# google/kubeflow

Measured on AMD Instinct MI355X. Metric: pytorchjob_train_tokens_per_s, higher is better.
Workload: dtype bf16; 1 GPU; model=llama3-8b, global_batch=7, seq_len=4096, parallelism=dp1

## Files before the change

### kubeflow_amd/ops/_backend.py

```python
from __future__ import annotations

import ctypes
import os
from pathlib import Path

_LIB_PATH = Path(__file__).resolve().parent / "libkfops.so"
_lib = None
_load_error: str | None = None


def native_enabled() -> bool:
    return os.environ.get("KF_NATIVE_KERNELS", "1") != "0"


def try_load():
    global _lib, _load_error
    if _lib is not None:
        return _lib
    if not native_enabled():
        _load_error = "disabled via KF_NATIVE_KERNELS=0"
        return None
    from . import build_ext
    if build_ext.needs_build():
        try:
# ... 27 lines not shown
_FP = ctypes.POINTER(ctypes.c_float)
_PI64 = ctypes.POINTER(ctypes.c_int64)
_PI32 = ctypes.POINTER(ctypes.c_int32)

_DQ8 = [_P] * 5 + [_FP, _FP] + [_I64] * 7 + [_F, _I32]
_DKV8 = [_P] + _DQ8
_ROPE_TAIL = [_FP, _FP, _I64]
_BWD_HEAD = [_P] * 8 + [_FP, _FP] + [_I64] * 4
_ATTN_BWD = _BWD_HEAD + [_I64] * 5 + [_F, _I32]
_ATTN_FWD = [_P, _FP, _P, _P, _P] + [_I64] * 7 + [_F, _I32, _P]

SIGNATURES: dict[str, list] = {
    "kf_rmsnorm_fwd": [_P, _FP, _P, _P, _I64, _I64, _F, _P],
    "kf_rmsnorm_bwd_nparts": [_I64],
    "kf_rmsnorm_bwd": [_P, _P, _FP, _P, _P, _P, _FP, _I64, _I64, _P],
    "kf_rmsnorm_bwd_res": [_P, _P, _FP, _P, _P, _P, _FP, _P, _I64, _I64, _P],
    "kf_layernorm_fwd": [_P, _FP, _FP, _P, _P, _P, _I64, _I64, _F, _P],
    "kf_layernorm_bwd_nparts": [_I64],
    "kf_layernorm_bwd": [_P, _P, _P, _FP, _P, _P, _P, _FP, _FP, _I64, _I64,
                         _P],
    "kf_rope": [_P, _P, _FP, _FP, _PI64] + [_I64] * 8 + [_I32, _P],
    "kf_swiglu_fwd": [_P, _P, _I64, _I64, _P],
    "kf_swiglu_bwd": [_P, _P, _P, _I64, _I64, _P],
    "kf_adamw": [_P, _FP, _P, _FP, _FP, _FP, _I64, _F, _F, _F, _F, _F, _I64,
                 _P],
    "kf_adamw_clip": [_P, _FP, _P, _FP, _FP, _FP, _P, _FP, _I64, _F, _F, _F,
                      _F, _F, _I64, _P],
    "kf_grad_sumsq_nparts": [_I64],
    "kf_grad_sumsq": [_FP, _FP, _P, _I64, _P],
    "kf_ce_fwd": [_FP, _FP, _P, _PI64, _I64, _I64, _I64, _P],
    "kf_ce_bwd": [_P, _P, _FP, _PI64, _FP, _I64, _I64, _I64, _P],
    "kf_skinny_gemm": [_P, _P, _P, _P] + [_I64] * 6 + [_P],
    "kf_skinny_gemm_q8": [_P, _P, _P, _FP, _P] + [_I64] * 6 + [_P],
    "kf_skinny_gemm_grouped": [_P, _P, _P, _PI32, _PI32] + [_I64] * 6 + [_P],
    "kf_skinny_gemm_grouped_q8": [_P, _P, _P, _FP, _PI32, _PI32] +
                                 [_I64] * 6 + [_P],
    "kf_kv_store": [_P] * 6 + [_I64, _I64, _I64, _P],
    "kf_decode_rope_store": [_P, _P, _P, _P, _FP, _FP, _PI32, _P] +
                            [_I64] * 5 + [_P],
    "kf_attn_fwd": _ATTN_FWD,
    "kf_attn_fwd4": _ATTN_FWD,
    "kf_attn_fwd4_rect": [_P, _FP, _P, _P, _P] + [_I64] * 8 + [_F, _I64, _P],
    "kf_attn_fwd4_abl": [_I32] + _ATTN_FWD,
    "kf_tr16_probe": [_P, _P, _I32, _P],
    "kf_attn_bwd": _ATTN_BWD + [_P],
    "kf_attn_bwd_rope": _ATTN_BWD + _ROPE_TAIL + [_P],
    "kf_attn_bwd8_dq": _DQ8 + [_P],
    "kf_attn_bwd8_dq_rope": _DQ8 + _ROPE_TAIL + [_P],
    "kf_attn_bwd8_dkv": _DKV8 + [_P],
    "kf_attn_bwd8_dkv_rope": _DKV8 + _ROPE_TAIL + [_P],
    "kf_attn_bwd8_dkv_fused": _DKV8 + [_P],
    "kf_attn_bwd8_dkv_fused_rope": _DKV8 + _ROPE_TAIL + [_P],
    "kf_attn64_fwd": [_P, _FP, _P, _P, _P] + [_I64] * 6 + [_F, _I32, _I64,
                                                           _P],
    "kf_attn64_bwd": _BWD_HEAD + [_I64, _I64, _F, _I32, _I64, _P],
    "kf_attn64_fwd_varlen": [_P, _FP, _P, _P, _P, _PI32] + [_I64] * 6 +
                            [_F, _P],
    "kf_attn64_bwd_varlen": _BWD_HEAD[:10] + [_PI32] + [_I64] * 6 + [_F, _P],
    "kf_attn_decode": [_P] * 6 + [_PI32, _PI32] + [_I64] * 6 + [_F, _P],
    "kf_moe_route": [_P, _FP, _P, _P, _I64, _I64, _I64, _P],
    "kf_moe_route_bwd": [_P, _P, _FP, _P, _I64, _I64, _I64, _P],
    "kf_moe_sort_nwork": [_I64, _I64, _I64],
    "kf_moe_sort": [_P] * 5 + [_I64] * 4 + [_P],
    "kf_moe_gather": [_P, _P, _P, _I64, _I64, _I64, _P],
    "kf_moe_gather_bwd": [_P, _P, _P] + [_I64] * 4 + [_P],
    "kf_moe_combine": [_P] * 4 + [_I64] * 4 + [_P],
    "kf_moe_combine_bwd": [_P] * 6 + [_I64] * 4 + [_P],
}
_RETURNS_INT64 = ("kf_rmsnorm_bwd_nparts", "kf_layernorm_bwd_nparts",
# ... 19 lines not shown
```

### kubeflow_amd/ops/csrc/attention_bwd.hip

```cpp

#include "kf_attn_common.h"

#define AB_D 128

__global__ __launch_bounds__(256) void kf_attn_delta2_kernel(
    float* __restrict__ delta, const unsigned short* __restrict__ dout,
    const unsigned short* __restrict__ o, int64_t B, int S, int Hq) {
  const int64_t nrows = B * (int64_t)S * Hq;
  const int wid = threadIdx.x / KF_WAVE;
  const int lane = threadIdx.x & (KF_WAVE - 1);
  for (int64_t row = blockIdx.x * 4 + wid; row < nrows; row += gridDim.x * 4) {
    const unsigned short* dor = dout + row * AB_D;
    const unsigned short* orow = o + row * AB_D;
    kf_short4 a = *reinterpret_cast<const kf_short4*>(dor + lane * 2);
    kf_short4 bv = *reinterpret_cast<const kf_short4*>(orow + lane * 2);
    float s = kf_bf16_to_f32((unsigned short)a[0]) *
                  kf_bf16_to_f32((unsigned short)bv[0]) +
              kf_bf16_to_f32((unsigned short)a[1]) *
                  kf_bf16_to_f32((unsigned short)bv[1]);
    s = kf_wave_sum(s);
    if (lane == 0) {
      const int h = (int)(row % Hq);
      const int64_t bs = row / Hq;
      const int64_t b = bs / S;
      const int st = (int)(bs % S);
      delta[(b * Hq + h) * (int64_t)S + st] = s;
    }
  }
}

#define DQ_KT 64

__global__ __launch_bounds__(256) void kf_attn_dq_kernel(
    unsigned short* __restrict__ dq, const unsigned short* __restrict__ q,
    const unsigned short* __restrict__ k, const unsigned short* __restrict__ v,
    const unsigned short* __restrict__ dout, const float* __restrict__ lse,
    const float* __restrict__ delta, int64_t B, int S, int Hq, int Hkv,
    int64_t qts, int64_t kts, int64_t dqts, float scale, int causal) {
  __shared__ unsigned char k_lds[DQ_KT * AB_D * 2];
  __shared__ unsigned char v_lds[DQ_KT * AB_D * 2];
  __shared__ unsigned char kt_lds[AB_D * DQ_KT * 2];
  __shared__ unsigned char ds_lds[4][16 * DQ_KT * 2];
// ... 243 lines not shown
      for (int nt = 0; nt < 8; ++nt) {
        kf_bf16x8 dob = *reinterpret_cast<const kf_bf16x8*>(
            dot_lds + kf_swz(nt * 16 + l16, lg * 16, 64));
        dvacc[nt] =
            __builtin_amdgcn_mfma_f32_16x16x32_bf16(ptf, dob, dvacc[nt], 0, 0, 0);
        kf_bf16x8 qb = *reinterpret_cast<const kf_bf16x8*>(
            qt_lds + kf_swz(nt * 16 + l16, lg * 16, 64));
        dkacc[nt] =
            __builtin_amdgcn_mfma_f32_16x16x32_bf16(dstf, qb, dkacc[nt], 0, 0, 0);
      }
    }
  }

  const int krow0 = kt * 64 + w * 16 + lg * 4;
#pragma unroll
  for (int r = 0; r < 4; ++r) {
    const int64_t base = (b * S + krow0 + r) * dkts + (int64_t)hkv * AB_D;
#pragma unroll
    for (int nt = 0; nt < 8; ++nt) {
      dk[base + nt * 16 + l16] = kf_f32_to_bf16(dkacc[nt][r]);
      dv[base + nt * 16 + l16] = kf_f32_to_bf16(dvacc[nt][r]);
    }
  }
}

KF_EXPORT int kf_attn_bwd(void* dq, void* dk, void* dv, const void* dout,
                          const void* q, const void* k, const void* v,
                          const void* o, const float* lse, float* delta,
                          int64_t B, int64_t S, int64_t Hq, int64_t Hkv,
                          int64_t D, int64_t qts, int64_t kts, int64_t dqts,
                          int64_t dkts, float scale, int causal,
                          void* stream) {
  return kf_attn_bwd_rope(dq, dk, dv, dout, q, k, v, o, lse, delta, B, S, Hq,
                          Hkv, D, qts, kts, dqts, dkts, scale, causal,
                          nullptr, nullptr, 0, stream);
}

KF_EXPORT int kf_attn_bwd_rope(void* dq, void* dk, void* dv, const void* dout,
                               const void* q, const void* k, const void* v,
                               const void* o, const float* lse, float* delta,
                               int64_t B, int64_t S, int64_t Hq, int64_t Hkv,
                               int64_t D, int64_t qts, int64_t kts,
                               int64_t dqts, int64_t dkts, float scale,
                               int causal, const float* cost,
                               const float* sint, int64_t pos_offset,
                               void* stream) {
  if (D != AB_D || S % 64 || Hq % Hkv) return (int)hipErrorInvalidValue;
  if ((cost == nullptr) != (sint == nullptr)) return (int)hipErrorInvalidValue;
  if (qts == 0) qts = Hq * AB_D;
  if (kts == 0) kts = Hkv * AB_D;
  if (dqts == 0) dqts = Hq * AB_D;
  if (dkts == 0) dkts = Hkv * AB_D;
  hipLaunchKernelGGL(kf_attn_delta2_kernel,
                     dim3(kf_grid_for(B * S * Hq, 4)), dim3(256), 0,
                     (hipStream_t)stream, delta, (const unsigned short*)dout,
                     (const unsigned short*)o, B, (int)S, (int)Hq);
  int err = (int)hipGetLastError();
  if (err) return err;
  if (S % 256 == 0) {
    err = kf_attn_bwd8_dq_rope(dq, q, k, v, dout, lse, delta, B, S, Hq, Hkv,
                               qts, kts, dqts, scale, causal, cost, sint,
                               pos_offset, stream);
    if (err) return err;
    return kf_attn_bwd8_dkv_fused_rope(dk, dv, q, k, v, dout, lse, delta, B,
                                       S, Hq, Hkv, qts, kts, dkts, scale,
                                       causal, cost, sint, pos_offset,
                                       stream);
  }
  dim3 gq((unsigned)(S / 64), (unsigned)Hq, (unsigned)B);
  hipLaunchKernelGGL(kf_attn_dq_kernel, gq, dim3(256), 0, (hipStream_t)stream,
                     (unsigned short*)dq, (const unsigned short*)q,
                     (const unsigned short*)k, (const unsigned short*)v,
                     (const unsigned short*)dout, lse, delta, B, (int)S,
                     (int)Hq, (int)Hkv, qts, kts, dqts, scale, causal);
  err = (int)hipGetLastError();
  if (err) return err;
  dim3 gkv((unsigned)(S / 64), (unsigned)Hkv, (unsigned)B);
  hipLaunchKernelGGL(kf_attn_dkv_kernel, gkv, dim3(256), 0,
                     (hipStream_t)stream, (unsigned short*)dk,
                     (unsigned short*)dv, (const unsigned short*)q,
                     (const unsigned short*)k, (const unsigned short*)v,
                     (const unsigned short*)dout, lse, delta, B, (int)S,
                     (int)Hq, (int)Hkv, qts, kts, dkts, scale, causal);
  err = (int)hipGetLastError();
  if (err || !cost) return err;
  return kf_rope(dq, dk, cost, sint, nullptr, B, S, Hq, Hkv, D, dqts, dkts,
                 pos_offset, 1, stream);
}
```

### kubeflow_amd/ops/csrc/attention_bwd8.hip

```cpp

#include "kf_attn_common.h"

#define AB_D 128

__device__ __forceinline__ int kf_subrow(int r, int byte_in_row) {
  return 2 * kf_vsub<64>(r, byte_in_row >> 1);
}

#define KF_ROPE_ADJ_PAIR(x1, x2, c, s)                                \
  {                                                                   \
    const float a_ = kf_bf16_to_f32(kf_f32_to_bf16(x1));              \
    const float b_ = kf_bf16_to_f32(kf_f32_to_bf16(x2));              \
    const float t1_ = b_ * (s), t2_ = a_ * (s);                       \
    (x1) = __builtin_fmaf(a_, (c), t1_);                              \
    (x2) = __builtin_fmaf(b_, (c), -t2_);                             \
  }

#define DQ8_QT 256
#define DQ8_KT 64

__global__ __launch_bounds__(512, 2) void kf_attn_dq8_kernel(
    unsigned short* __restrict__ dq, const unsigned short* __restrict__ q,
    const unsigned short* __restrict__ k, const unsigned short* __restrict__ v,
    const unsigned short* __restrict__ dout, const float* __restrict__ lse,
    const float* __restrict__ delta, int64_t B, int S, int Hq, int Hkv,
    int64_t qts, int64_t kts, int64_t dqts, float scale, int causal,
    const float* __restrict__ cost, const float* __restrict__ sint,
    int64_t pos_offset) {
  __shared__ unsigned char k_lds[2][DQ8_KT * AB_D * 2];
  __shared__ unsigned char v_lds[2][DQ8_KT * AB_D * 2];

  const int nqt = gridDim.x / (Hq * (int)B);
  const int qt = causal ? (nqt - 1 - blockIdx.x / (Hq * (int)B))
                        : (int)(blockIdx.x / (Hq * (int)B));
  const int rest = blockIdx.x % (Hq * (int)B);
  const int hq = rest % Hq;
  const int64_t b = rest / Hq;
  const int hkv = hq / (Hq / Hkv);
  const int tid = threadIdx.x;
  const int w = tid / KF_WAVE;
  const int lane = tid & 63, l31 = lane & 31, hi = lane >> 5;
  const int qrow_g = qt * DQ8_QT + w * 32 + l31;
  const int wave_qmax = qt * DQ8_QT + w * 32 + 31;
  const float scale2 = scale * KF_LOG2E;

  kf_bf16x8 qfrag[8], dofrag[8];
  {
    const int64_t qb = (b * S + qrow_g) * qts + (int64_t)hq * AB_D;
    const int64_t db = ((b * S + qrow_g) * (int64_t)Hq + hq) * AB_D;
#pragma unroll
    for (int kk = 0; kk < 8; ++kk) {
      qfrag[kk] =
          *reinterpret_cast<const kf_bf16x8*>(q + qb + kk * 16 + hi * 8);
      dofrag[kk] =
          *reinterpret_cast<const kf_bf16x8*>(dout + db + kk * 16 + hi * 8);
    }
  }
  const float lse2_q =
      lse[(b * Hq + hq) * (int64_t)S + qrow_g] * KF_LOG2E;
  const float dlt_q = delta[(b * Hq + hq) * (int64_t)S + qrow_g];

  kf_f32x16 dqacc[4];
#pragma unroll
  for (int i = 0; i < 4; ++i) dqacc[i] = kf_f32x16{0.f};

  const unsigned short* kg0 = k + (b * S) * kts + (int64_t)hkv * AB_D;
  const unsigned short* vg0 = v + (b * S) * kts + (int64_t)hkv * AB_D;
  const int sr0 = tid >> 4, sr1 = (tid + 512) >> 4, c8 = tid & 15;
  const unsigned tr_off = kf_tr_lane_off<64>(lane);

  const int last_kt =
      causal ? (qt * DQ8_QT + DQ8_QT - 1) / DQ8_KT : (S / DQ8_KT - 1);

  kf_short8 kst0, kst1, vst0, vst1;
  kst0 = *reinterpret_cast<const kf_short8*>(kg0 + sr0 * kts + c8 * 8);
  kst1 = *reinterpret_cast<const kf_short8*>(kg0 + sr1 * kts + c8 * 8);
  vst0 = *reinterpret_cast<const kf_short8*>(vg0 + sr0 * kts + c8 * 8);
  vst1 = *reinterpret_cast<const kf_short8*>(vg0 + sr1 * kts + c8 * 8);
  auto stage_write = [&](int buf) {
    *reinterpret_cast<kf_short8*>(k_lds[buf] + 2 * kf_vsub<64>(sr0, c8 * 8)) =
        kst0;
    *reinterpret_cast<kf_short8*>(k_lds[buf] + 2 * kf_vsub<64>(sr1, c8 * 8)) =
        kst1;
// ... 571 lines not shown
        KF_ROPE_ADJ_PAIR(dkacc[dt][r], dkacc[dt + 2][r], cost[cb + dt * 32],
                         sint[cb + dt * 32]);
    }
#pragma unroll
    for (int dt = 0; dt < 4; ++dt)
      dk[base + dt * 32 + l31] = kf_f32_to_bf16(dkacc[dt][r]);
  }
}

KF_EXPORT int kf_attn_bwd8_dq_rope(void* dq, const void* q, const void* k,
                                   const void* v, const void* dout,
                                   const float* lse, const float* delta,
                                   int64_t B, int64_t S, int64_t Hq,
                                   int64_t Hkv, int64_t qts, int64_t kts,
                                   int64_t dqts, float scale, int causal,
                                   const float* cost, const float* sint,
                                   int64_t pos_offset, void* stream) {
  dim3 gq((unsigned)((S / DQ8_QT) * Hq * B), 1, 1);
  hipLaunchKernelGGL(kf_attn_dq8_kernel, gq, dim3(512), 0,
                     (hipStream_t)stream, (unsigned short*)dq,
                     (const unsigned short*)q, (const unsigned short*)k,
                     (const unsigned short*)v, (const unsigned short*)dout,
                     lse, delta, B, (int)S, (int)Hq, (int)Hkv, qts, kts, dqts,
                     scale, causal, cost, sint, pos_offset);
  return (int)hipGetLastError();
}

KF_EXPORT int kf_attn_bwd8_dq(void* dq, const void* q, const void* k,
                              const void* v, const void* dout,
                              const float* lse, const float* delta, int64_t B,
                              int64_t S, int64_t Hq, int64_t Hkv, int64_t qts,
                              int64_t kts, int64_t dqts, float scale,
                              int causal, void* stream) {
  return kf_attn_bwd8_dq_rope(dq, q, k, v, dout, lse, delta, B, S, Hq, Hkv,
                              qts, kts, dqts, scale, causal, nullptr, nullptr,
                              0, stream);
}

KF_EXPORT int kf_attn_bwd8_dkv_rope(void* dk, void* dv, const void* q,
                                    const void* k, const void* v,
                                    const void* dout, const float* lse,
                                    const float* delta, int64_t B, int64_t S,
                                    int64_t Hq, int64_t Hkv, int64_t qts,
                                    int64_t kts, int64_t dkts, float scale,
                                    int causal, const float* cost,
                                    const float* sint, int64_t pos_offset,
                                    void* stream) {
// ... 58 lines not shown
```

### kubeflow_amd/ops/csrc/kf_common.h

```cpp
#pragma once

#include <hip/hip_runtime.h>
#include <hip/hip_bf16.h>
#include <cstdint>

#define KF_WAVE 64

#include "kf_ops.h"

typedef short kf_short4 __attribute__((ext_vector_type(4)));
typedef short kf_short8 __attribute__((ext_vector_type(8)));
typedef float kf_float4 __attribute__((ext_vector_type(4)));

__device__ __forceinline__ float kf_bf16_to_f32(unsigned short u) {
  union { float f; unsigned int i; } w;
  w.i = ((unsigned int)u) << 16;
  return w.f;
}

__device__ __forceinline__ unsigned short kf_f32_to_bf16(float f) {
  union { float f; unsigned int i; } w;
  w.f = f;
  unsigned int x = w.i;
  if ((x & 0x7FFFFFFFu) > 0x7F800000u) return 0x7FC0;
  unsigned int rounding = 0x7fff + ((x >> 16) & 1);
  x += rounding;
  return (unsigned short)(x >> 16);
}

__device__ __forceinline__ float kf_wave_sum(float v) {
#pragma unroll
  for (int off = 32; off > 0; off >>= 1) v += __shfl_xor(v, off, KF_WAVE);
  return v;
}

__device__ __forceinline__ float kf_wave_max(float v) {
#pragma unroll
  for (int off = 32; off > 0; off >>= 1) v = fmaxf(v, __shfl_xor(v, off, KF_WAVE));
  return v;
}

template <typename Op>
__device__ __forceinline__ float kf_block_reduce(float v, float* scratch, Op op,
                                                 float init) {
  const int lane = threadIdx.x & (KF_WAVE - 1);
  const int wid = threadIdx.x / KF_WAVE;
  const int nw = blockDim.x / KF_WAVE;
#pragma unroll
  for (int off = 32; off > 0; off >>= 1) v = op(v, __shfl_xor(v, off, KF_WAVE));
  if (lane == 0) scratch[wid] = v;
// ... 17 lines not shown
```

### kubeflow_amd/ops/csrc/kf_ops.h

```cpp
#pragma once

#include <cstdint>

#define KF_EXPORT extern "C" __attribute__((visibility("default")))

KF_EXPORT int kf_rmsnorm_fwd(void* y, float* rstd, const void* x,
    const void* w, int64_t rows, int64_t cols, float eps, void* stream);
KF_EXPORT int64_t kf_rmsnorm_bwd_nparts(int64_t rows);
KF_EXPORT int kf_rmsnorm_bwd(void* dx, void* dw, float* dw_acc, const void* dy,
    const void* x, const void* w, const float* rstd, int64_t rows,
    int64_t cols, void* stream);
KF_EXPORT int kf_rmsnorm_bwd_res(void* dx, void* dw, float* dw_acc,
    const void* dy, const void* x, const void* w, const float* rstd,
    const void* dres, int64_t rows, int64_t cols, void* stream);
KF_EXPORT int kf_layernorm_fwd(void* y, float* mu, float* rstd, const void* x,
    const void* w, const void* b, int64_t rows, int64_t cols, float eps,
    void* stream);
KF_EXPORT int64_t kf_layernorm_bwd_nparts(int64_t rows);
KF_EXPORT int kf_layernorm_bwd(void* dx, void* dw, void* db, float* part,
    const void* dy, const void* x, const void* w, const float* mu,
    const float* rstd, int64_t rows, int64_t cols, void* stream);

KF_EXPORT int kf_rope(void* q, void* k, const float* cost, const float* sint,
    const int64_t* positions, int64_t B, int64_t S, int64_t Hq, int64_t Hkv,
    int64_t D, int64_t qts, int64_t kts, int64_t pos_offset, int backward,
    void* stream);
KF_EXPORT int kf_swiglu_fwd(void* y, const void* h, int64_t T, int64_t F,
    void* stream);
KF_EXPORT int kf_swiglu_bwd(void* dh, const void* dy, const void* h, int64_t T,
    int64_t F, void* stream);
KF_EXPORT int kf_adamw(void* p16, float* p32, const void* g, float* m,
    float* v, const float* wd_mask, int64_t n, float lr, float b1, float b2,
    float eps, float wd, int64_t step, void* stream);
KF_EXPORT int kf_adamw_clip(void* p16, float* p32, void* g, float* m,
    float* v, const float* wd_mask, const void* wd_groups,
    const float* gscale, int64_t n, float lr, float b1, float b2, float eps,
    float wd, int64_t step, void* stream);
KF_EXPORT int64_t kf_grad_sumsq_nparts(int64_t n);
KF_EXPORT int kf_grad_sumsq(float* out, float* partials, const void* g,
    int64_t n, void* stream);
KF_EXPORT int kf_ce_fwd(float* loss_sum, float* lse, const void* logits,
    const int64_t* targets, int64_t T, int64_t V, int64_t ignore_index,
    void* stream);
KF_EXPORT int kf_ce_bwd(void* dlogits, const void* logits, const float* lse,
    const int64_t* targets, const float* scale, int64_t T, int64_t V,
    int64_t ignore_index, void* stream);

KF_EXPORT int kf_skinny_gemm(void* c, const void* a, const void* w,
    const void* res, int64_t M, int64_t N, int64_t K, int64_t lda,
    int64_t ldw, int64_t ldc, void* stream);
KF_EXPORT int kf_skinny_gemm_q8(void* c, const void* a, const void* w8,
    const float* wscale, const void* res, int64_t M, int64_t N, int64_t K,
    int64_t lda, int64_t ldw, int64_t ldc, void* stream);
// ... 20 lines not shown
    const void* v, int64_t B, int64_t S, int64_t Hq, int64_t Hkv, int64_t D,
    int64_t qts, int64_t kts, float scale, int causal, void* stream);
KF_EXPORT int kf_attn_fwd4_rect(void* o, float* lse, const void* q,
    const void* k, const void* v, int64_t B, int64_t Sq, int64_t Skv,
    int64_t Hq, int64_t Hkv, int64_t D, int64_t qts, int64_t kts, float scale,
    int64_t qoff, void* stream);
KF_EXPORT int kf_attn_fwd4_abl(int mode, void* o, float* lse, const void* q,
    const void* k, const void* v, int64_t B, int64_t S, int64_t Hq,
    int64_t Hkv, int64_t D, int64_t qts, int64_t kts, float scale, int causal,
    void* stream);
KF_EXPORT int kf_tr16_probe(void* out, const void* in, int mode, void* stream);

KF_EXPORT int kf_attn_bwd(void* dq, void* dk, void* dv, const void* dout,
    const void* q, const void* k, const void* v, const void* o,
    const float* lse, float* delta, int64_t B, int64_t S, int64_t Hq,
    int64_t Hkv, int64_t D, int64_t qts, int64_t kts, int64_t dqts,
    int64_t dkts, float scale, int causal, void* stream);
KF_EXPORT int kf_attn_bwd_rope(void* dq, void* dk, void* dv, const void* dout,
    const void* q, const void* k, const void* v, const void* o,
    const float* lse, float* delta, int64_t B, int64_t S, int64_t Hq,
    int64_t Hkv, int64_t D, int64_t qts, int64_t kts, int64_t dqts,
    int64_t dkts, float scale, int causal, const float* cost,
    const float* sint, int64_t pos_offset, void* stream);
KF_EXPORT int kf_attn_bwd8_dq(void* dq, const void* q, const void* k,
    const void* v, const void* dout, const float* lse, const float* delta,
    int64_t B, int64_t S, int64_t Hq, int64_t Hkv, int64_t qts, int64_t kts,
    int64_t dqts, float scale, int causal, void* stream);
KF_EXPORT int kf_attn_bwd8_dq_rope(void* dq, const void* q, const void* k,
    const void* v, const void* dout, const float* lse, const float* delta,
    int64_t B, int64_t S, int64_t Hq, int64_t Hkv, int64_t qts, int64_t kts,
    int64_t dqts, float scale, int causal, const float* cost,
    const float* sint, int64_t pos_offset, void* stream);
KF_EXPORT int kf_attn_bwd8_dkv(void* dk, void* dv, const void* q,
    const void* k, const void* v, const void* dout, const float* lse,
    const float* delta, int64_t B, int64_t S, int64_t Hq, int64_t Hkv,
    int64_t qts, int64_t kts, int64_t dkts, float scale, int causal,
    void* stream);
KF_EXPORT int kf_attn_bwd8_dkv_rope(void* dk, void* dv, const void* q,
    const void* k, const void* v, const void* dout, const float* lse,
    const float* delta, int64_t B, int64_t S, int64_t Hq, int64_t Hkv,
    int64_t qts, int64_t kts, int64_t dkts, float scale, int causal,
    const float* cost, const float* sint, int64_t pos_offset, void* stream);
KF_EXPORT int kf_attn_bwd8_dkv_fused(void* dk, void* dv, const void* q,
    const void* k, const void* v, const void* dout, const float* lse,
    const float* delta, int64_t B, int64_t S, int64_t Hq, int64_t Hkv,
    int64_t qts, int64_t kts, int64_t dkts, float scale, int causal,
// ... 50 lines not shown
```

### kubeflow_amd/ops/csrc/rope.hip

```cpp

#include "kf_common.h"

#define ROPE_VEC 4

__global__ void kf_rope_kernel(unsigned short* __restrict__ q,
                               unsigned short* __restrict__ k,
                               const float* __restrict__ cost,
                               const float* __restrict__ sint,
                               const int64_t* __restrict__ positions,
                               int64_t B, int S, int Hq, int Hkv, int D,
                               int64_t qts, int64_t kts,
                               int64_t pos_offset, int backward) {
  const int Ht = Hq + Hkv;
  const int halfD = D / 2;
  const int quads = halfD / ROPE_VEC;
  const int64_t total = B * (int64_t)S * Ht * quads;
  for (int64_t it = blockIdx.x * (int64_t)blockDim.x + threadIdx.x; it < total;
       it += gridDim.x * (int64_t)blockDim.x) {
    const int qd = (int)(it % quads);
    int64_t rest = it / quads;
    const int h = (int)(rest % Ht);
    rest /= Ht;
    const int s = (int)(rest % S);
    const int64_t b = rest / S;
    unsigned short* base;
    if (h < Hq) base = q + (b * S + s) * qts + (int64_t)h * D;
    else base = k + (b * S + s) * kts + (int64_t)(h - Hq) * D;
    const int d0 = qd * ROPE_VEC;
    kf_short4 x1 = *reinterpret_cast<const kf_short4*>(base + d0);
    kf_short4 x2 = *reinterpret_cast<const kf_short4*>(base + halfD + d0);
    const int64_t pos = (positions ? positions[b] : pos_offset) + s;
    kf_float4 c = *reinterpret_cast<const kf_float4*>(
        cost + pos * (int64_t)halfD + d0);
    kf_float4 sn = *reinterpret_cast<const kf_float4*>(
        sint + pos * (int64_t)halfD + d0);
    kf_short4 o1, o2;
#pragma unroll
    for (int j = 0; j < ROPE_VEC; ++j) {
      float a = kf_bf16_to_f32((unsigned short)x1[j]);
      float bb = kf_bf16_to_f32((unsigned short)x2[j]);
      float sj = backward ? -sn[j] : sn[j];
      o1[j] = (short)kf_f32_to_bf16(a * c[j] - bb * sj);
      o2[j] = (short)kf_f32_to_bf16(bb * c[j] + a * sj);
    }
    *reinterpret_cast<kf_short4*>(base + d0) = o1;
    *reinterpret_cast<kf_short4*>(base + halfD + d0) = o2;
  }
}

KF_EXPORT int kf_rope(void* q, void* k, const float* cost, const float* sint,
                      const int64_t* positions, int64_t B, int64_t S,
                      int64_t Hq, int64_t Hkv, int64_t D, int64_t qts,
                      int64_t kts, int64_t pos_offset, int backward,
                      void* stream) {
  if ((D / 2) % ROPE_VEC) return (int)hipErrorInvalidValue;
  const int64_t total = B * S * (Hq + Hkv) * (D / 2 / ROPE_VEC);
  hipLaunchKernelGGL(kf_rope_kernel, dim3(kf_grid_for(total, 256)), dim3(256),
                     0, (hipStream_t)stream, (unsigned short*)q,
                     (unsigned short*)k, cost, sint, positions, B, (int)S,
                     (int)Hq, (int)Hkv, (int)D, qts, kts, pos_offset,
                     backward);
  return (int)hipGetLastError();
}
```

### kubeflow_amd/ops/csrc/swiglu.hip

```cpp

#include "kf_common.h"

__device__ __forceinline__ float kf_sigmoid(float x) {
  return 1.f / (1.f + __expf(-x));
}

__global__ void kf_swiglu_fwd_kernel(unsigned short* __restrict__ y,
                                     const unsigned short* __restrict__ h,
                                     int64_t T, int64_t F) {
  const int64_t nvec = T * F / 8;
  for (int64_t i = blockIdx.x * (int64_t)blockDim.x + threadIdx.x; i < nvec;
       i += gridDim.x * (int64_t)blockDim.x) {
    const int64_t t = (i * 8) / F;
    const int64_t f = (i * 8) % F;
    kf_short8 gv = *reinterpret_cast<const kf_short8*>(h + t * 2 * F + f);
    kf_short8 uv = *reinterpret_cast<const kf_short8*>(h + t * 2 * F + F + f);
    kf_short8 ov;
#pragma unroll
    for (int j = 0; j < 8; ++j) {
      float g = kf_bf16_to_f32((unsigned short)gv[j]);
      float u = kf_bf16_to_f32((unsigned short)uv[j]);
      ov[j] = (short)kf_f32_to_bf16(g * kf_sigmoid(g) * u);
    }
    *reinterpret_cast<kf_short8*>(y + t * F + f) = ov;
  }
}

__global__ void kf_swiglu_bwd_kernel(unsigned short* __restrict__ dh,
                                     const unsigned short* __restrict__ dy,
                                     const unsigned short* __restrict__ h,
                                     int64_t T, int64_t F) {
  const int64_t nvec = T * F / 8;
  for (int64_t i = blockIdx.x * (int64_t)blockDim.x + threadIdx.x; i < nvec;
       i += gridDim.x * (int64_t)blockDim.x) {
    const int64_t t = (i * 8) / F;
    const int64_t f = (i * 8) % F;
    kf_short8 gv = *reinterpret_cast<const kf_short8*>(h + t * 2 * F + f);
    kf_short8 uv = *reinterpret_cast<const kf_short8*>(h + t * 2 * F + F + f);
    kf_short8 dyv = *reinterpret_cast<const kf_short8*>(dy + t * F + f);
    kf_short8 dgv, duv;
#pragma unroll
    for (int j = 0; j < 8; ++j) {
      float g = kf_bf16_to_f32((unsigned short)gv[j]);
      float u = kf_bf16_to_f32((unsigned short)uv[j]);
      float d = kf_bf16_to_f32((unsigned short)dyv[j]);
      float sig = kf_sigmoid(g);
      float silu = g * sig;
      dgv[j] = (short)kf_f32_to_bf16(d * u * (sig + silu * (1.f - sig)));
      duv[j] = (short)kf_f32_to_bf16(d * silu);
    }
    *reinterpret_cast<kf_short8*>(dh + t * 2 * F + f) = dgv;
    *reinterpret_cast<kf_short8*>(dh + t * 2 * F + F + f) = duv;
  }
}

KF_EXPORT int kf_swiglu_fwd(void* y, const void* h, int64_t T, int64_t F,
                            void* stream) {
  if (F % 8) return (int)hipErrorInvalidValue;
  hipLaunchKernelGGL(kf_swiglu_fwd_kernel, dim3(kf_grid_for(T * F / 8, 256)),
                     dim3(256), 0, (hipStream_t)stream, (unsigned short*)y,
                     (const unsigned short*)h, T, F);
  return (int)hipGetLastError();
}

KF_EXPORT int kf_swiglu_bwd(void* dh, const void* dy, const void* h,
                            int64_t T, int64_t F, void* stream) {
  if (F % 8) return (int)hipErrorInvalidValue;
  hipLaunchKernelGGL(kf_swiglu_bwd_kernel, dim3(kf_grid_for(T * F / 8, 256)),
                     dim3(256), 0, (hipStream_t)stream, (unsigned short*)dh,
                     (const unsigned short*)dy, (const unsigned short*)h, T, F);
  return (int)hipGetLastError();
}
```

Baseline: 21630 tokens/s.

## Fold attention delta into dq backward kernel and rewrite rope/swiglu kernels

Computes the attention backward delta (rowsum of dout*o) inside the dq kernel for the S%256 path, removing a separate delta launch and its extra read of dout/o. Rewrites RoPE as a per-token kernel that loads cos/sin once and loops over heads with wider vector loads. Rewrites SwiGLU forward/backward as per-row kernels using 128-bit packed bf16 words and hardware bf16 conversion. Keeps the old kernels as _ref exports; the dkv kernel must read delta written by the dq kernel, which relies on stream ordering.

Result: no change. 21730 tokens/s, median of 6 (+0.5%).

```diff
diff --git a/kubeflow_amd/ops/_backend.py b/kubeflow_amd/ops/_backend.py
--- a/kubeflow_amd/ops/_backend.py
+++ b/kubeflow_amd/ops/_backend.py
@@ -73,6 +73,9 @@
     "kf_rope": [_P, _P, _FP, _FP, _PI64] + [_I64] * 8 + [_I32, _P],
     "kf_swiglu_fwd": [_P, _P, _I64, _I64, _P],
     "kf_swiglu_bwd": [_P, _P, _P, _I64, _I64, _P],
+    "kf_rope_ref": [_P, _P, _FP, _FP, _PI64] + [_I64] * 8 + [_I32, _P],
+    "kf_swiglu_fwd_ref": [_P, _P, _I64, _I64, _P],
+    "kf_swiglu_bwd_ref": [_P, _P, _P, _I64, _I64, _P],
     "kf_adamw": [_P, _FP, _P, _FP, _FP, _FP, _I64, _F, _F, _F, _F, _F, _I64,
                  _P],
     "kf_adamw_clip": [_P, _FP, _P, _FP, _FP, _FP, _P, _FP, _I64, _F, _F, _F,
@@ -96,6 +99,9 @@
     "kf_tr16_probe": [_P, _P, _I32, _P],
     "kf_attn_bwd": _ATTN_BWD + [_P],
     "kf_attn_bwd_rope": _ATTN_BWD + _ROPE_TAIL + [_P],
+    "kf_attn_delta": [_FP, _P, _P, _I64, _I64, _I64, _P],
+    "kf_attn_bwd8_dq_fold_rope": [_P] * 6 + [_FP, _FP] + [_I64] * 7 +
+                                 [_F, _I32] + _ROPE_TAIL + [_P],
     "kf_attn_bwd8_dq": _DQ8 + [_P],
     "kf_attn_bwd8_dq_rope": _DQ8 + _ROPE_TAIL + [_P],
     "kf_attn_bwd8_dkv": _DKV8 + [_P],
diff --git a/kubeflow_amd/ops/csrc/attention_bwd.hip b/kubeflow_amd/ops/csrc/attention_bwd.hip
--- a/kubeflow_amd/ops/csrc/attention_bwd.hip
+++ b/kubeflow_amd/ops/csrc/attention_bwd.hip
@@ -12,12 +12,11 @@
   for (int64_t row = blockIdx.x * 4 + wid; row < nrows; row += gridDim.x * 4) {
     const unsigned short* dor = dout + row * AB_D;
     const unsigned short* orow = o + row * AB_D;
-    kf_short4 a = *reinterpret_cast<const kf_short4*>(dor + lane * 2);
-    kf_short4 bv = *reinterpret_cast<const kf_short4*>(orow + lane * 2);
-    float s = kf_bf16_to_f32((unsigned short)a[0]) *
-                  kf_bf16_to_f32((unsigned short)bv[0]) +
-              kf_bf16_to_f32((unsigned short)a[1]) *
-                  kf_bf16_to_f32((unsigned short)bv[1]);
+    const unsigned int a =
+        *reinterpret_cast<const unsigned int*>(dor + lane * 2);
+    const unsigned int bv =
+        *reinterpret_cast<const unsigned int*>(orow + lane * 2);
+    float s = kf_bf16_lo(a) * kf_bf16_lo(bv) + kf_bf16_hi(a) * kf_bf16_hi(bv);
     s = kf_wave_sum(s);
     if (lane == 0) {
       const int h = (int)(row % Hq);
@@ -307,6 +306,15 @@
       dv[base + nt * 16 + l16] = kf_f32_to_bf16(dvacc[nt][r]);
     }
   }
+}
+
+KF_EXPORT int kf_attn_delta(float* delta, const void* dout, const void* o,
+                            int64_t B, int64_t S, int64_t Hq, void* stream) {
+  hipLaunchKernelGGL(kf_attn_delta2_kernel,
+                     dim3(kf_grid_for(B * S * Hq, 4)), dim3(256), 0,
+                     (hipStream_t)stream, delta, (const unsigned short*)dout,
+                     (const unsigned short*)o, B, (int)S, (int)Hq);
+  return (int)hipGetLastError();
 }
 
 KF_EXPORT int kf_attn_bwd(void* dq, void* dk, void* dv, const void* dout,
@@ -336,22 +344,19 @@
   if (kts == 0) kts = Hkv * AB_D;
   if (dqts == 0) dqts = Hq * AB_D;
   if (dkts == 0) dkts = Hkv * AB_D;
-  hipLaunchKernelGGL(kf_attn_delta2_kernel,
-                     dim3(kf_grid_for(B * S * Hq, 4)), dim3(256), 0,
-                     (hipStream_t)stream, delta, (const unsigned short*)dout,
-                     (const unsigned short*)o, B, (int)S, (int)Hq);
-  int err = (int)hipGetLastError();
-  if (err) return err;
+  int err;
   if (S % 256 == 0) {
-    err = kf_attn_bwd8_dq_rope(dq, q, k, v, dout, lse, delta, B, S, Hq, Hkv,
-                               qts, kts, dqts, scale, causal, cost, sint,
-                               pos_offset, stream);
+    err = kf_attn_bwd8_dq_fold_rope(dq, q, k, v, dout, o, lse, delta, B, S,
+                                    Hq, Hkv, qts, kts, dqts, scale, causal,
+                                    cost, sint, pos_offset, stream);
     if (err) return err;
     return kf_attn_bwd8_dkv_fused_rope(dk, dv, q, k, v, dout, lse, delta, B,
                                        S, Hq, Hkv, qts, kts, dkts, scale,
                                        causal, cost, sint, pos_offset,
                                        stream);
   }
+  err = kf_attn_delta(delta, dout, o, B, S, Hq, stream);
+  if (err) return err;
   dim3 gq((unsigned)(S / 64), (unsigned)Hq, (unsigned)B);
   hipLaunchKernelGGL(kf_attn_dq_kernel, gq, dim3(256), 0, (hipStream_t)stream,
                      (unsigned short*)dq, (const unsigned short*)q,
diff --git a/kubeflow_amd/ops/csrc/attention_bwd8.hip b/kubeflow_amd/ops/csrc/attention_bwd8.hip
--- a/kubeflow_amd/ops/csrc/attention_bwd8.hip
+++ b/kubeflow_amd/ops/csrc/attention_bwd8.hip
@@ -26,7 +26,8 @@
     const float* __restrict__ delta, int64_t B, int S, int Hq, int Hkv,
     int64_t qts, int64_t kts, int64_t dqts, float scale, int causal,
     const float* __restrict__ cost, const float* __restrict__ sint,
-    int64_t pos_offset) {
+    int64_t pos_offset, const unsigned short* __restrict__ o,
+    float* __restrict__ delta_out) {
   __shared__ unsigned char k_lds[2][DQ8_KT * AB_D * 2];
   __shared__ unsigned char v_lds[2][DQ8_KT * AB_D * 2];
 
@@ -45,9 +46,9 @@
   const float scale2 = scale * KF_LOG2E;
 
   kf_bf16x8 qfrag[8], dofrag[8];
+  const int64_t db = ((b * S + qrow_g) * (int64_t)Hq + hq) * AB_D;
   {
     const int64_t qb = (b * S + qrow_g) * qts + (int64_t)hq * AB_D;
-    const int64_t db = ((b * S + qrow_g) * (int64_t)Hq + hq) * AB_D;
 #pragma unroll
     for (int kk = 0; kk < 8; ++kk) {
       qfrag[kk] =
@@ -56,9 +57,32 @@
           *reinterpret_cast<const kf_bf16x8*>(dout + db + kk * 16 + hi * 8);
     }
   }
-  const float lse2_q =
-      lse[(b * Hq + hq) * (int64_t)S + qrow_g] * KF_LOG2E;
-  const float dlt_q = delta[(b * Hq + hq) * (int64_t)S + qrow_g];
+  const int64_t rowc = (b * Hq + hq) * (int64_t)S + qrow_g;
+  const float lse2_q = lse[rowc] * KF_LOG2E;
+  float dlt_q;
+  if (o) {
+    float p[8][4];
+#pragma unroll
+    for (int kk = 0; kk < 8; ++kk) {
+      const kf_bf16x8 ov =
+          *reinterpret_cast<const kf_bf16x8*>(o + db + kk * 16 + hi * 8);
+#pragma unroll
+      for (int j = 0; j < 4; ++j)
+        p[kk][j] = (float)dofrag[kk][2 * j] * (float)ov[2 * j] +
+                   (float)dofrag[kk][2 * j + 1] * (float)ov[2 * j + 1];
+    }
+    float a[4];
+#pragma unroll
+    for (int j = 0; j < 4; ++j) {
+      a[j] = ((p[0][j] + p[4][j]) + (p[2][j] + p[6][j])) +
+             ((p[1][j] + p[5][j]) + (p[3][j] + p[7][j]));
+      a[j] += __shfl_xor(a[j], 32, KF_WAVE);
+    }
+    dlt_q = (a[0] + a[2]) + (a[1] + a[3]);
+    if (hi == 0) delta_out[rowc] = dlt_q;
+  } else {
+    dlt_q = delta[rowc];
+  }
 
   kf_f32x16 dqacc[4];
 #pragma unroll
@@ -676,7 +700,27 @@
                      (const unsigned short*)q, (const unsigned short*)k,
                      (const unsigned short*)v, (const unsigned short*)dout,
                      lse, delta, B, (int)S, (int)Hq, (int)Hkv, qts, kts, dqts,
-                     scale, causal, cost, sint, pos_offset);
+                     scale, causal, cost, sint, pos_offset,
+                     (const unsigned short*)nullptr, (float*)nullptr);
+  return (int)hipGetLastError();
+}
+
+KF_EXPORT int kf_attn_bwd8_dq_fold_rope(
+    void* dq, const void* q, const void* k, const void* v, const void* dout,
+    const void* o, const float* lse, float* delta_out, int64_t B, int64_t S,
+    int64_t Hq, int64_t Hkv, int64_t qts, int64_t kts, int64_t dqts,
+    float scale, int causal, const float* cost, const float* sint,
+    int64_t pos_offset, void* stream) {
+  if (!o || !delta_out || S % DQ8_QT || Hq % Hkv)
+    return (int)hipErrorInvalidValue;
+  dim3 gq((unsigned)((S / DQ8_QT) * Hq * B), 1, 1);
+  hipLaunchKernelGGL(kf_attn_dq8_kernel, gq, dim3(512), 0,
+                     (hipStream_t)stream, (unsigned short*)dq,
+                     (const unsigned short*)q, (const unsigned short*)k,
+                     (const unsigned short*)v, (const unsigned short*)dout,
+                     lse, (const float*)nullptr, B, (int)S, (int)Hq, (int)Hkv,
+                     qts, kts, dqts, scale, causal, cost, sint, pos_offset,
+                     (const unsigned short*)o, delta_out);
   return (int)hipGetLastError();
 }
 
diff --git a/kubeflow_amd/ops/csrc/kf_common.h b/kubeflow_amd/ops/csrc/kf_common.h
--- a/kubeflow_amd/ops/csrc/kf_common.h
+++ b/kubeflow_amd/ops/csrc/kf_common.h
@@ -26,6 +26,21 @@
   unsigned int rounding = 0x7fff + ((x >> 16) & 1);
   x += rounding;
   return (unsigned short)(x >> 16);
+}
+
+typedef unsigned int kf_uint2 __attribute__((ext_vector_type(2)));
+typedef unsigned int kf_uint4 __attribute__((ext_vector_type(4)));
+typedef __bf16 kf_bf16pair __attribute__((ext_vector_type(2)));
+
+__device__ __forceinline__ float kf_bf16_lo(unsigned int w) {
+  return __builtin_bit_cast(float, w << 16);
+}
+__device__ __forceinline__ float kf_bf16_hi(unsigned int w) {
+  return __builtin_bit_cast(float, w & 0xFFFF0000u);
+}
+__device__ __forceinline__ unsigned int kf_pack_bf16(float lo, float hi) {
+  kf_bf16pair p = {(__bf16)lo, (__bf16)hi};
+  return __builtin_bit_cast(unsigned int, p);
 }
 
 __device__ __forceinline__ float kf_wave_sum(float v) {
diff --git a/kubeflow_amd/ops/csrc/kf_ops.h b/kubeflow_amd/ops/csrc/kf_ops.h
--- a/kubeflow_amd/ops/csrc/kf_ops.h
+++ b/kubeflow_amd/ops/csrc/kf_ops.h
@@ -29,6 +29,14 @@
     void* stream);
 KF_EXPORT int kf_swiglu_bwd(void* dh, const void* dy, const void* h, int64_t T,
     int64_t F, void* stream);
+KF_EXPORT int kf_rope_ref(void* q, void* k, const float* cost,
+    const float* sint, const int64_t* positions, int64_t B, int64_t S,
+    int64_t Hq, int64_t Hkv, int64_t D, int64_t qts, int64_t kts,
+    int64_t pos_offset, int backward, void* stream);
+KF_EXPORT int kf_swiglu_fwd_ref(void* y, const void* h, int64_t T, int64_t F,
+    void* stream);
+KF_EXPORT int kf_swiglu_bwd_ref(void* dh, const void* dy, const void* h,
+    int64_t T, int64_t F, void* stream);
 KF_EXPORT int kf_adamw(void* p16, float* p32, const void* g, float* m,
     float* v, const float* wd_mask, int64_t n, float lr, float b1, float b2,
     float eps, float wd, int64_t step, void* stream);
@@ -95,6 +103,13 @@
     int64_t Hkv, int64_t D, int64_t qts, int64_t kts, int64_t dqts,
     int64_t dkts, float scale, int causal, const float* cost,
     const float* sint, int64_t pos_offset, void* stream);
+KF_EXPORT int kf_attn_delta(float* delta, const void* dout, const void* o,
+    int64_t B, int64_t S, int64_t Hq, void* stream);
+KF_EXPORT int kf_attn_bwd8_dq_fold_rope(void* dq, const void* q, const void* k,
+    const void* v, const void* dout, const void* o, const float* lse,
+    float* delta_out, int64_t B, int64_t S, int64_t Hq, int64_t Hkv,
+    int64_t qts, int64_t kts, int64_t dqts, float scale, int causal,
+    const float* cost, const float* sint, int64_t pos_offset, void* stream);
 KF_EXPORT int kf_attn_bwd8_dq(void* dq, const void* q, const void* k,
     const void* v, const void* dout, const float* lse, const float* delta,
     int64_t B, int64_t S, int64_t Hq, int64_t Hkv, int64_t qts, int64_t kts,
diff --git a/kubeflow_amd/ops/csrc/rope.hip b/kubeflow_amd/ops/csrc/rope.hip
--- a/kubeflow_amd/ops/csrc/rope.hip
+++ b/kubeflow_amd/ops/csrc/rope.hip
@@ -3,14 +3,14 @@
 
 #define ROPE_VEC 4
 
-__global__ void kf_rope_kernel(unsigned short* __restrict__ q,
-                               unsigned short* __restrict__ k,
-                               const float* __restrict__ cost,
-                               const float* __restrict__ sint,
-                               const int64_t* __restrict__ positions,
-                               int64_t B, int S, int Hq, int Hkv, int D,
-                               int64_t qts, int64_t kts,
-                               int64_t pos_offset, int backward) {
+__global__ void kf_rope_ref_kernel(unsigned short* __restrict__ q,
+                                   unsigned short* __restrict__ k,
+                                   const float* __restrict__ cost,
+                                   const float* __restrict__ sint,
+                                   const int64_t* __restrict__ positions,
+                                   int64_t B, int S, int Hq, int Hkv, int D,
+                                   int64_t qts, int64_t kts,
+                                   int64_t pos_offset, int backward) {
   const int Ht = Hq + Hkv;
   const int halfD = D / 2;
   const int quads = halfD / ROPE_VEC;
@@ -48,15 +48,127 @@
   }
 }
 
+#define ROPE_MAX_THREADS 512
+
+template <int VEC> struct kf_rope_words;
+template <> struct kf_rope_words<4> { typedef kf_uint2 type; };
+template <> struct kf_rope_words<8> { typedef kf_uint4 type; };
+
+__device__ __forceinline__ void kf_rope_pair(float& o1, float& o2, float a,
+                                             float b, float c, float sj) {
+  const float t1 = b * sj, t2 = a * sj;
+  o1 = __builtin_fmaf(a, c, -t1);
+  o2 = __builtin_fmaf(b, c, t2);
+}
+
+template <int VEC>
+__global__ __launch_bounds__(ROPE_MAX_THREADS) void kf_rope_kernel(
+    unsigned short* __restrict__ q, unsigned short* __restrict__ k,
+    const float* __restrict__ cost, const float* __restrict__ sint,
+    const int64_t* __restrict__ positions, int64_t B, int S, int Hq, int Hkv,
+    int D, int64_t qts, int64_t kts, int64_t pos_offset, int backward) {
+  typedef typename kf_rope_words<VEC>::type words_t;
+  const int Ht = Hq + Hkv;
+  const int halfD = D / 2;
+  const int chunks = halfD / VEC;
+  for (int64_t b = blockIdx.y; b < B; b += gridDim.y) {
+    const int64_t pos0 = positions ? positions[b] : pos_offset;
+    for (int s = blockIdx.x; s < S; s += gridDim.x) {
+      const int64_t tok = b * S + s;
+      unsigned short* qtok = q + tok * qts;
+      unsigned short* ktok = k + tok * kts;
+      const float* ctok = cost + (pos0 + s) * (int64_t)halfD;
+      const float* stok = sint + (pos0 + s) * (int64_t)halfD;
+      for (int ch = threadIdx.x; ch < chunks; ch += blockDim.x) {
+        const int d0 = ch * VEC;
+        float c[VEC], sj[VEC];
+#pragma unroll
+        for (int i = 0; i < VEC / 4; ++i) {
+          const kf_float4 c4 =
+              *reinterpret_cast<const kf_float4*>(ctok + d0 + 4 * i);
+          const kf_float4 s4 =
+              *reinterpret_cast<const kf_float4*>(stok + d0 + 4 * i);
+#pragma unroll
+          for (int j = 0; j < 4; ++j) {
+            c[4 * i + j] = c4[j];
+            sj[4 * i + j] = backward ? -s4[j] : s4[j];
+          }
+        }
+        for (int h = threadIdx.y; h < Ht; h += blockDim.y) {
+          unsigned short* base = (h < Hq ? qtok + (int64_t)h * D
+                                         : ktok + (int64_t)(h - Hq) * D) + d0;
+          const words_t x1 = *reinterpret_cast<const words_t*>(base);
+          const words_t x2 = *reinterpret_cast<const words_t*>(base + halfD);
+          words_t y1, y2;
+#pragma unroll
+          for (int j = 0; j < VEC / 2; ++j) {
+            float o1l, o2l, o1h, o2h;
+            kf_rope_pair(o1l, o2l, kf_bf16_lo(x1[j]), kf_bf16_lo(x2[j]),
+                         c[2 * j], sj[2 * j]);
+            kf_rope_pair(o1h, o2h, kf_bf16_hi(x1[j]), kf_bf16_hi(x2[j]),
+                         c[2 * j + 1], sj[2 * j + 1]);
+            y1[j] = kf_pack_bf16(o1l, o1h);
+            y2[j] = kf_pack_bf16(o2l, o2h);
+          }
+          *reinterpret_cast<words_t*>(base) = y1;
+          *reinterpret_cast<words_t*>(base + halfD) = y2;
+        }
+      }
+    }
+  }
+}
+
+static inline bool kf_rope_dims_ok(int64_t B, int64_t S, int64_t Hq,
+                                   int64_t Hkv, int64_t D) {
+  const int64_t lim = 0x7FFFFFFF;
+  return B >= 0 && S >= 0 && Hq >= 0 && Hkv >= 0 && D >= 0 && S <= lim &&
+         Hq + Hkv <= lim && D <= lim && (D / 2) % ROPE_VEC == 0 && D % 2 == 0;
+}
+
 KF_EXPORT int kf_rope(void* q, void* k, const float* cost, const float* sint,
                       const int64_t* positions, int64_t B, int64_t S,
                       int64_t Hq, int64_t Hkv, int64_t D, int64_t qts,
                       int64_t kts, int64_t pos_offset, int backward,
                       void* stream) {
+  if (!kf_rope_dims_ok(B, S, Hq, Hkv, D)) return (int)hipErrorInvalidValue;
+  if (B == 0 || S == 0 || Hq + Hkv == 0 || D == 0) return (int)hipSuccess;
+  const bool wide = (D / 2) % 8 == 0 && qts % 8 == 0 && kts % 8 == 0 &&
+                    (((uintptr_t)q | (uintptr_t)k) & 15) == 0;
+  const int64_t chunks = D / 2 / (wide ? 8 : ROPE_VEC);
+  const int bx = (int)(chunks < ROPE_MAX_THREADS ? chunks : ROPE_MAX_THREADS);
+  const int64_t max_y = ROPE_MAX_THREADS / bx;
+  const int64_t passes = (Hq + Hkv + max_y - 1) / max_y;
+  const int by = (int)((Hq + Hkv + passes - 1) / passes);
+  int64_t cap = (int64_t)2048 * 256 / (bx * by);
+  if (cap < 1) cap = 1;
+  const int64_t gx = S < cap ? S : cap;
+  int64_t gy = cap / gx;
+  if (gy > B) gy = B;
+  if (gy > 65535) gy = 65535;
+  if (gy < 1) gy = 1;
+  const dim3 grid((unsigned)gx, (unsigned)gy), block(bx, by);
+  if (wide)
+    hipLaunchKernelGGL(kf_rope_kernel<8>, grid, block, 0, (hipStream_t)stream,
+                       (unsigned short*)q, (unsigned short*)k, cost, sint,
+                       positions, B, (int)S, (int)Hq, (int)Hkv, (int)D, qts,
+                       kts, pos_offset, backward);
+  else
+    hipLaunchKernelGGL(kf_rope_kernel<4>, grid, block, 0, (hipStream_t)stream,
+                       (unsigned short*)q, (unsigned short*)k, cost, sint,
+                       positions, B, (int)S, (int)Hq, (int)Hkv, (int)D, qts,
+                       kts, pos_offset, backward);
+  return (int)hipGetLastError();
+}
+
+KF_EXPORT int kf_rope_ref(void* q, void* k, const float* cost,
+                          const float* sint, const int64_t* positions,
+                          int64_t B, int64_t S, int64_t Hq, int64_t Hkv,
+                          int64_t D, int64_t qts, int64_t kts,
+                          int64_t pos_offset, int backward, void* stream) {
   if ((D / 2) % ROPE_VEC) return (int)hipErrorInvalidValue;
   const int64_t total = B * S * (Hq + Hkv) * (D / 2 / ROPE_VEC);
-  hipLaunchKernelGGL(kf_rope_kernel, dim3(kf_grid_for(total, 256)), dim3(256),
-                     0, (hipStream_t)stream, (unsigned short*)q,
+  hipLaunchKernelGGL(kf_rope_ref_kernel, dim3(kf_grid_for(total, 256)),
+                     dim3(256), 0, (hipStream_t)stream, (unsigned short*)q,
                      (unsigned short*)k, cost, sint, positions, B, (int)S,
                      (int)Hq, (int)Hkv, (int)D, qts, kts, pos_offset,
                      backward);
diff --git a/kubeflow_amd/ops/csrc/swiglu.hip b/kubeflow_amd/ops/csrc/swiglu.hip
--- a/kubeflow_amd/ops/csrc/swiglu.hip
+++ b/kubeflow_amd/ops/csrc/swiglu.hip
@@ -1,13 +1,27 @@
 
 #include "kf_common.h"
+
+#define SWIGLU_THREADS 256
 
 __device__ __forceinline__ float kf_sigmoid(float x) {
   return 1.f / (1.f + __expf(-x));
 }
 
-__global__ void kf_swiglu_fwd_kernel(unsigned short* __restrict__ y,
-                                     const unsigned short* __restrict__ h,
-                                     int64_t T, int64_t F) {
+__device__ __forceinline__ float kf_swiglu_y(float g, float u) {
+  return g * kf_sigmoid(g) * u;
+}
+
+__device__ __forceinline__ void kf_swiglu_grad(float& dg, float& du, float g,
+                                               float u, float d) {
+  float sig = kf_sigmoid(g);
+  float silu = g * sig;
+  dg = d * u * (sig + silu * (1.f - sig));
+  du = d * silu;
+}
+
+__global__ void kf_swiglu_fwd_ref_kernel(unsigned short* __restrict__ y,
+                                         const unsigned short* __restrict__ h,
+                                         int64_t T, int64_t F) {
   const int64_t nvec = T * F / 8;
   for (int64_t i = blockIdx.x * (int64_t)blockDim.x + threadIdx.x; i < nvec;
        i += gridDim.x * (int64_t)blockDim.x) {
@@ -20,16 +34,16 @@
     for (int j = 0; j < 8; ++j) {
       float g = kf_bf16_to_f32((unsigned short)gv[j]);
       float u = kf_bf16_to_f32((unsigned short)uv[j]);
-      ov[j] = (short)kf_f32_to_bf16(g * kf_sigmoid(g) * u);
+      ov[j] = (short)kf_f32_to_bf16(kf_swiglu_y(g, u));
     }
     *reinterpret_cast<kf_short8*>(y + t * F + f) = ov;
   }
 }
 
-__global__ void kf_swiglu_bwd_kernel(unsigned short* __restrict__ dh,
-                                     const unsigned short* __restrict__ dy,
-                                     const unsigned short* __restrict__ h,
-                                     int64_t T, int64_t F) {
+__global__ void kf_swiglu_bwd_ref_kernel(unsigned short* __restrict__ dh,
+                                         const unsigned short* __restrict__ dy,
+                                         const unsigned short* __restrict__ h,
+                                         int64_t T, int64_t F) {
   const int64_t nvec = T * F / 8;
   for (int64_t i = blockIdx.x * (int64_t)blockDim.x + threadIdx.x; i < nvec;
        i += gridDim.x * (int64_t)blockDim.x) {
@@ -44,30 +58,134 @@
       float g = kf_bf16_to_f32((unsigned short)gv[j]);
       float u = kf_bf16_to_f32((unsigned short)uv[j]);
       float d = kf_bf16_to_f32((unsigned short)dyv[j]);
-      float sig = kf_sigmoid(g);
-      float silu = g * sig;
-      dgv[j] = (short)kf_f32_to_bf16(d * u * (sig + silu * (1.f - sig)));
-      duv[j] = (short)kf_f32_to_bf16(d * silu);
+      float dg, du;
+      kf_swiglu_grad(dg, du, g, u, d);
+      dgv[j] = (short)kf_f32_to_bf16(dg);
+      duv[j] = (short)kf_f32_to_bf16(du);
     }
     *reinterpret_cast<kf_short8*>(dh + t * 2 * F + f) = dgv;
     *reinterpret_cast<kf_short8*>(dh + t * 2 * F + F + f) = duv;
   }
 }
 
+__device__ __forceinline__ kf_uint4 kf_swiglu_fwd_vec(kf_uint4 g, kf_uint4 u) {
+  kf_uint4 y;
+#pragma unroll
+  for (int j = 0; j < 4; ++j)
+    y[j] = kf_pack_bf16(kf_swiglu_y(kf_bf16_lo(g[j]), kf_bf16_lo(u[j])),
+                        kf_swiglu_y(kf_bf16_hi(g[j]), kf_bf16_hi(u[j])));
+  return y;
+}
+
+__device__ __forceinline__ void kf_swiglu_bwd_vec(kf_uint4& dg, kf_uint4& du,
+                                                  kf_uint4 g, kf_uint4 u,
+                                                  kf_uint4 d) {
+#pragma unroll
+  for (int j = 0; j < 4; ++j) {
+    float dg0, du0, dg1, du1;
+    kf_swiglu_grad(dg0, du0, kf_bf16_lo(g[j]), kf_bf16_lo(u[j]),
+                   kf_bf16_lo(d[j]));
+    kf_swiglu_grad(dg1, du1, kf_bf16_hi(g[j]), kf_bf16_hi(u[j]),
+                   kf_bf16_hi(d[j]));
+    dg[j] = kf_pack_bf16(dg0, dg1);
+    du[j] = kf_pack_bf16(du0, du1);
+  }
+}
+
+__global__ __launch_bounds__(SWIGLU_THREADS) void kf_swiglu_fwd_kernel(
+    unsigned short* __restrict__ y, const unsigned short* __restrict__ h,
+    int64_t T, int64_t F) {
+  const int nv = (int)(F / 8);
+  for (int64_t t = blockIdx.x; t < T; t += gridDim.x) {
+    const kf_uint4* __restrict__ g =
+        reinterpret_cast<const kf_uint4*>(h + t * 2 * F);
+    const kf_uint4* __restrict__ u = g + nv;
+    kf_uint4* __restrict__ yr = reinterpret_cast<kf_uint4*>(y + t * F);
+    int v = threadIdx.x;
+    for (; v + SWIGLU_THREADS < nv; v += 2 * SWIGLU_THREADS) {
+      const kf_uint4 g0 = g[v], u0 = u[v];
+      const kf_uint4 g1 = g[v + SWIGLU_THREADS], u1 = u[v + SWIGLU_THREADS];
+      yr[v] = kf_swiglu_fwd_vec(g0, u0);
+      yr[v + SWIGLU_THREADS] = kf_swiglu_fwd_vec(g1, u1);
+    }
+    if (v < nv) yr[v] = kf_swiglu_fwd_vec(g[v], u[v]);
+  }
+}
+
+__global__ __launch_bounds__(SWIGLU_THREADS) void kf_swiglu_bwd_kernel(
+    unsigned short* __restrict__ dh, const unsigned short* __restrict__ dy,
+    const unsigned short* __restrict__ h, int64_t T, int64_t F) {
+  const int nv = (int)(F / 8);
+  for (int64_t t = blockIdx.x; t < T; t += gridDim.x) {
+    const kf_uint4* __restrict__ g =
+        reinterpret_cast<const kf_uint4*>(h + t * 2 * F);
+    const kf_uint4* __restrict__ u = g + nv;
+    const kf_uint4* __restrict__ d =
+        reinterpret_cast<const kf_uint4*>(dy + t * F);
+    kf_uint4* __restrict__ dgr = reinterpret_cast<kf_uint4*>(dh + t * 2 * F);
+    kf_uint4* __restrict__ dur = dgr + nv;
+    int v = threadIdx.x;
+    for (; v + SWIGLU_THREADS < nv; v += 2 * SWIGLU_THREADS) {
+      const kf_uint4 g0 = g[v], u0 = u[v], d0 = d[v];
+      const kf_uint4 g1 = g[v + SWIGLU_THREADS], u1 = u[v + SWIGLU_THREADS],
+                     d1 = d[v + SWIGLU_THREADS];
+      kf_uint4 dg, du;
+      kf_swiglu_bwd_vec(dg, du, g0, u0, d0);
+      dgr[v] = dg;
+      dur[v] = du;
+      kf_swiglu_bwd_vec(dg, du, g1, u1, d1);
+      dgr[v + SWIGLU_THREADS] = dg;
+      dur[v + SWIGLU_THREADS] = du;
+    }
+    if (v < nv) {
+      kf_uint4 dg, du;
+      kf_swiglu_bwd_vec(dg, du, g[v], u[v], d[v]);
+      dgr[v] = dg;
+      dur[v] = du;
+    }
+  }
+}
+
+static inline bool kf_swiglu_dims_ok(int64_t T, int64_t F) {
+  return T >= 0 && F >= 0 && F % 8 == 0 &&
+         F / 8 <= 0x7FFFFFFF - 4 * SWIGLU_THREADS;
+}
+
 KF_EXPORT int kf_swiglu_fwd(void* y, const void* h, int64_t T, int64_t F,
                             void* stream) {
-  if (F % 8) return (int)hipErrorInvalidValue;
-  hipLaunchKernelGGL(kf_swiglu_fwd_kernel, dim3(kf_grid_for(T * F / 8, 256)),
-                     dim3(256), 0, (hipStream_t)stream, (unsigned short*)y,
-                     (const unsigned short*)h, T, F);
+  if (!kf_swiglu_dims_ok(T, F)) return (int)hipErrorInvalidValue;
+  hipLaunchKernelGGL(kf_swiglu_fwd_kernel, dim3(kf_grid_for(T, 1)),
+                     dim3(SWIGLU_THREADS), 0, (hipStream_t)stream,
+                     (unsigned short*)y, (const unsigned short*)h, T, F);
   return (int)hipGetLastError();
 }
 
 KF_EXPORT int kf_swiglu_bwd(void* dh, const void* dy, const void* h,
                             int64_t T, int64_t F, void* stream) {
+  if (!kf_swiglu_dims_ok(T, F)) return (int)hipErrorInvalidValue;
+  hipLaunchKernelGGL(kf_swiglu_bwd_kernel, dim3(kf_grid_for(T, 1)),
+                     dim3(SWIGLU_THREADS), 0, (hipStream_t)stream,
+                     (unsigned short*)dh, (const unsigned short*)dy,
+                     (const unsigned short*)h, T, F);
+  return (int)hipGetLastError();
+}
+
+KF_EXPORT int kf_swiglu_fwd_ref(void* y, const void* h, int64_t T, int64_t F,
+                                void* stream) {
   if (F % 8) return (int)hipErrorInvalidValue;
-  hipLaunchKernelGGL(kf_swiglu_bwd_kernel, dim3(kf_grid_for(T * F / 8, 256)),
-                     dim3(256), 0, (hipStream_t)stream, (unsigned short*)dh,
+  hipLaunchKernelGGL(kf_swiglu_fwd_ref_kernel,
+                     dim3(kf_grid_for(T * F / 8, 256)), dim3(256), 0,
+                     (hipStream_t)stream, (unsigned short*)y,
+                     (const unsigned short*)h, T, F);
+  return (int)hipGetLastError();
+}
+
+KF_EXPORT int kf_swiglu_bwd_ref(void* dh, const void* dy, const void* h,
+                                int64_t T, int64_t F, void* stream) {
+  if (F % 8) return (int)hipErrorInvalidValue;
+  hipLaunchKernelGGL(kf_swiglu_bwd_ref_kernel,
+                     dim3(kf_grid_for(T * F / 8, 256)), dim3(256), 0,
+                     (hipStream_t)stream, (unsigned short*)dh,
                      (const unsigned short*)dy, (const unsigned short*)h, T, F);
   return (int)hipGetLastError();
 }
```
